# zhexin1904/gtsam_personal

Hardware: AMD Instinct MI355X
Metric: LM iterations/sec (higher is better)
Workload: dtype f64; 1 GPU; synthetic BAL 1000 cameras / 100000 points / 1000002 factors (GeneralSFMFactor<Cal3Bundler> + 2 priors), seed 42, METIS ordering (Ordering::Metis of the reference, fixture-carried permutation), LM legacy defaults; ordering=metis, cameras=1000, points=100000, factors=1000002, fronts=100001, parallelism=single GPU

## Files before the change

gtsam_personal_amd/_lib.py:

```python
from __future__ import annotations

import ctypes as ct
import os

_HERE = os.path.dirname(os.path.abspath(__file__))
LIB_PATH = os.path.join(_HERE, "liblmgpu.so")

LMGPU_OK, LMGPU_INDETERMINATE, LMGPU_INVALID, LMGPU_HIP_ERROR = 0, 1, 2, 3


class lmgpu_config(ct.Structure):
    _fields_ = [("device", ct.c_int32), ("rank", ct.c_int32), ("world_size", ct.c_int32), ("flags", ct.c_int32)]


class lmgpu_lm_params(ct.Structure):
    _fields_ = [
        ("maxIterations", ct.c_int32),
        ("relativeErrorTol", ct.c_double), ("absoluteErrorTol", ct.c_double), ("errorTol", ct.c_double),
        ("lambdaInitial", ct.c_double), ("lambdaFactor", ct.c_double), ("lambdaUpperBound", ct.c_double), ("lambdaLowerBound", ct.c_double),
        ("minModelFidelity", ct.c_double),
        ("diagonalDamping", ct.c_int32), ("useFixedLambdaFactor", ct.c_int32),
        ("minDiagonal", ct.c_double), ("maxDiagonal", ct.c_double),
    ]

# ... 128 lines not shown
    "lmgpu_init_pose3_num_factors": (ct.c_int, [_H]),
    "lmgpu_init_pose3_get_slots": (ct.c_int, [_H, ct.POINTER(ct.c_uint64)]),
    "lmgpu_init_pose3_handle": (ct.c_void_p, [_H, ct.c_int32]),
    "lmgpu_init_pose3_orientations_chordal": (ct.c_int, [_H, _D]),
    "lmgpu_init_pose3_closest_rotations": (ct.c_int, [ct.c_int32, ct.c_int32, _D, _D]),
    "lmgpu_init_pose3_orientations_gradient": (ct.c_int, [_H, _D, ct.c_int32, ct.c_int32, _D, _I, _D]),
    "lmgpu_init_pose3_compute_poses": (ct.c_int, [_H, _D, ct.c_int32, _D, ct.POINTER(lmgpu_lm_state)]),
    "lmgpu_init_pose3_initialize": (ct.c_int, [_H, _D, ct.c_int32, _D]),
    "lmgpu_set_kernel_timing": (ct.c_int, [_H, ct.c_int32]),
    "lmgpu_get_kernel_times": (ct.c_int, [_H, _D, _D, ct.POINTER(ct.c_int64)]),
    "lmgpu_get_jacobian": (ct.c_int, [_H, ct.c_int32, _D, _I, _I]),
    "lmgpu_get_jacobians": (ct.c_int, [_H, _I, _I, _I, _I, ct.POINTER(ct.c_int64), _D]),
    "lmgpu_num_fronts": (ct.c_int, [_H]),
    "lmgpu_front_info": (ct.c_int, [_H, ct.c_int32, _I]),
    "lmgpu_leaf_group_launches": (ct.c_int, [_H]),
    "lmgpu_backsub_group_launches": (ct.c_int, [_H, _I]),
    "lmgpu_get_leaf_corner": (ct.c_int, [_H, ct.c_int32, _D]),
    "lmgpu_get_front": (ct.c_int, [_H, ct.c_int32, _I, _D]),
    "lmgpu_comm_unique_id": (ct.c_int, [ct.c_char_p]),
    "lmgpu_comm_init": (ct.c_int, [_H, ct.c_char_p]),
    "lmgpu_marginal_covariance": (ct.c_int, [_H, ct.c_int32, _D]),
    "lmgpu_joint_marginal_covariance": (ct.c_int, [_H, ct.c_int32, _I, _D]),
    "lmgpu_selftest_chain_schedule": (ct.c_int, [ct.c_int, ct.c_int, ct.c_int, ct.c_int, ct.c_int]),
    "lmgpu_selftest_dense_schedule": (ct.c_int, [ct.c_int, ct.c_int, ct.c_int, ct.c_uint, ct.c_int, _I]),
    "lmgpu_selftest_dogleg_step": (ct.c_int, [ct.c_int, _D, _D]),
    "lmgpu_bt_products": (ct.c_int, [_H, _D, ct.c_double, _D, _D]),
    "lmgpu_isam2_create": (ct.c_int, [ct.POINTER(lmgpu_config), ct.c_void_p, ct.c_void_p, ct.c_void_p, ct.POINTER(_H)]),
    "lmgpu_isam2_destroy": (ct.c_int, [_H]),
    "lmgpu_isam2_last_error": (ct.c_char_p, [_H]),
    "lmgpu_isam2_last_failed_key": (ct.c_uint64, [_H]),
# ... 90 lines not shown
```

gtsam_personal_amd/csrc/kernels_potrf.hpp:

```cpp
#pragma once
#include <hip/hip_runtime.h>

namespace lmgpu {

typedef double double4_t __attribute__((ext_vector_type(4)));

__device__ __forceinline__ double readlane_d(double v, int src_lane) {
  const long long b = __double_as_longlong(v);
  const int lo = __builtin_amdgcn_readlane((int)(b & 0xffffffffLL), src_lane);
  const int hi = __builtin_amdgcn_readlane((int)(b >> 32), src_lane);
  return __longlong_as_double(((long long)hi << 32) | (unsigned int)lo);
}

__device__ __forceinline__ double fast_rsqrt(double p) {
  double y = __builtin_amdgcn_rsq(p);
  const double h = 0.5 * p;
  y = y * fma(-h * y, y, 1.5);
  y = y * fma(-h * y, y, 1.5);
  return y;
}

template <bool INV>
__device__ __forceinline__ bool potrf64_wave_g4(double4_t (&T)[4][4], double4_t (&E)[4], int nrows = 64) {
  const int lane = threadIdx.x & 63, kk = lane >> 4, cc = lane & 15;
  bool failed = false;
#pragma unroll
  for (int g = 0; g < 4; g++) {
    if (INV) {
#pragma unroll
      for (int r = 0; r < 4; r++) E[g][r] = (kk + 4 * r == cc) ? 1.0 : 0.0;
    }
    if (16 * g >= nrows) continue;
#pragma unroll
    for (int q = 0; q < 4; q++) {
      if (16 * g + 4 * q >= nrows) continue;
      double m[4][4];
#pragma unroll
      for (int a = 0; a < 4; a++)
#pragma unroll
        for (int b = a; b < 4; b++) m[a][b] = readlane_d(T[g][g][q], 16 * a + 4 * q + b);
      double R[4][4], inv[4];
#pragma unroll
      for (int a = 0; a < 4; a++) {
        double p = m[a][a];
#pragma unroll
        for (int k = 0; k < a; k++) p -= R[k][a] * R[k][a];
        const bool pok = p > 0.0;
        failed |= !pok;
        p = pok ? p : 1.0;
        const double rs = fast_rsqrt(p);
        inv[a] = rs;
        R[a][a] = p * rs;
#pragma unroll
        for (int b = a + 1; b < 4; b++) {
          double v = m[a][b];
#pragma unroll
          for (int k = 0; k < a; k++) v -= R[k][a] * R[k][b];
          R[a][b] = v * rs;
        }
      }
      double W[4][4];
#pragma unroll
      for (int a = 0; a < 4; a++) {
        W[a][a] = inv[a];
#pragma unroll
        for (int b = a + 1; b < 4; b++) {
          double v = 0;
#pragma unroll
          for (int k = a; k < b; k++) v += W[a][k] * R[k][b];
          W[a][b] = -v * inv[b];
        }
      }
      double aop = 0.0;
#pragma unroll
      for (int k = 0; k < 4; k++)
#pragma unroll
        for (int i = k; i < 4; i++) aop = (kk == k && cc == i) ? W[k][i] : aop;
      double bop = 0.0;
      {
        const double4_t x = __builtin_amdgcn_mfma_f64_16x16x4f64(aop, T[g][g][q], double4_t{0, 0, 0, 0}, 0, 0, 0);
        T[g][g][q] = x[0];
        if (q < 3) {
          bop = (cc >= 4 * (q + 1)) ? -T[g][g][q] : 0.0;
          T[g][g] = __builtin_amdgcn_mfma_f64_16x16x4f64(bop, T[g][g][q], T[g][g], 0, 0, 0);
        }
      }
#pragma unroll
      for (int h = g + 1; h < 4; h++) {
        const double4_t x = __builtin_amdgcn_mfma_f64_16x16x4f64(aop, T[g][h][q], double4_t{0, 0, 0, 0}, 0, 0, 0);
        T[g][h][q] = x[0];
        if (q < 3) T[g][h] = __builtin_amdgcn_mfma_f64_16x16x4f64(bop, T[g][h][q], T[g][h], 0, 0, 0);
      }
      if (INV) {
        const double4_t x = __builtin_amdgcn_mfma_f64_16x16x4f64(aop, E[g][q], double4_t{0, 0, 0, 0}, 0, 0, 0);
        E[g][q] = x[0];
        if (q < 3) E[g] = __builtin_amdgcn_mfma_f64_16x16x4f64(bop, E[g][q], E[g], 0, 0, 0);
      }
    }
#pragma unroll
    for (int g2 = g + 1; g2 < 4; g2++)
#pragma unroll
      for (int h = g2; h < 4; h++)
#pragma unroll
        for (int s = 0; s < 4; s++) T[g2][h] = __builtin_amdgcn_mfma_f64_16x16x4f64(-T[g][g2][s], T[g][h][s], T[g2][h], 0, 0, 0);
  }
  return failed;
}
__device__ __forceinline__ bool potrf64_wave_g4(double4_t (&T)[4][4]) {
  double4_t E[4];
  return potrf64_wave_g4<false>(T, E);
}

#define DP_LDW 66
#define DIAG_LDS_DOUBLES (64 * DP_LDW + 4 * 16 * 17 + 3 * 64 * DP_LDW)
#define DIAG_LDS_BYTES (DIAG_LDS_DOUBLES * 8)

__device__ __forceinline__ int frexp_exp_d(double x) {
  int e;
  frexp(x, &e);
// ... 206 lines not shown
          const int row = 16 * g + kk + 4 * r;
          if (row < nbj && cvalid) P[(size_t)(64 * j + row) * ld + c0 + cc] = out[r];
        }
      }
    }
  }
}

__global__ __launch_bounds__(256) void panel_trsm_kernel(double* __restrict__ A, int ld, int n, int ko, int kb, const double* __restrict__ inv16) {
  __shared__ double I16[16][16][17];
  panel_trsm_body(A, ld, n, ko, kb, inv16, I16, blockIdx.x);
}

#define TAIL_MAX_M 48
#define TAIL_MAX_KP 256
#define TAIL_LDS_BYTES ((TAIL_MAX_KP * TAIL_MAX_M + TAIL_MAX_M * TAIL_MAX_M + 64 * 65) * 8)
__global__ __launch_bounds__(256) void front_tail_kernel(double* __restrict__ A, int ld, int n, int nf, int p0, int kp, int front_id,
                                                         int* __restrict__ status, double* __restrict__ inv16) {
  extern __shared__ double tsm[];
  const int r0 = p0 + kp, m = n - r0, nft = nf - r0, tid = threadIdx.x;
  double* Pl = tsm;
  double* S = tsm + (size_t)TAIL_MAX_KP * TAIL_MAX_M;
  double(*D)[65] = (double(*)[65])(S + TAIL_MAX_M * TAIL_MAX_M);
  for (int idx = tid; idx < kp * m; idx += 256) {
    const int k = idx / m, j = idx - k * m;
    Pl[idx] = A[(size_t)(p0 + k) * ld + r0 + j];
  }
  for (int idx = tid; idx < m * m; idx += 256) {
    const int i = idx / m, j = idx - i * m;
    S[idx] = (j >= i) ? A[(size_t)(r0 + i) * ld + r0 + j] : 0.0;
  }
  __syncthreads();
  for (int idx = tid; idx < m * m; idx += 256) {
// ... 50 lines not shown
  __syncthreads();
  if (tid < 64) {
    const int blk = tid >> 4, c = tid & 15, base = 16 * blk;
    double x[16];
#pragma unroll
    for (int i = 15; i >= 0; i--) {
      double sacc = (i == c) ? 1.0 : 0.0;
#pragma unroll
      for (int kq = i + 1; kq < 16; kq++) sacc -= D[base + i][base + kq] * x[kq];
      x[i] = (i <= c) ? sacc / D[base + i][base + i] : 0.0;
    }
#pragma unroll
    for (int i = 0; i < 16; i++) inv16[(size_t)blk * 256 + i * 16 + c] = x[i];
  }
}

#ifndef PDF_STAMP
#define PDF_STAMP(flags, b, slot)
#endif
#define PDF_TA0 32
#define PDF_MAX_COLTILES 992
#define PDF_PR0 1024
#define PDF_TD0 1536
#define PDF_FLAG_WORDS 8192
#define PDF_MAX_CHAIN_T 114
#define PDF_SPIN_LIMIT 2000000L
#define PDF_LDS_DOUBLES (2 * 64 * DP_LDW)
#define PDF_LDS_BYTES (PDF_LDS_DOUBLES * 8)

__host__ __device__ inline unsigned int pdf_ta_need(int sj) { return sj < 4 ? 4u * (unsigned int)(sj + 1) : 2u; }
// ... 264 lines not shown
```

gtsam_personal_amd/csrc/lmgpu.hip:

```cpp
#include <hip/hip_runtime.h>
#include <rccl/rccl.h>

#include <algorithm>
#include <chrono>
#include <cmath>
#include <cstdio>
#include <cstdlib>
#include <cstring>
#include <condition_variable>
#include <limits>
#include <mutex>
#include <string>
#include <map>
#include <vector>

#include "../../include/lmgpu.h"
#include "kernels_dense.hpp"
#include "kernels_potrf.hpp"
#include "kernels_step.hpp"
#include "dense_schedule.hpp"
#include "dogleg_step.hpp"
#include "kernels_batched.hpp"
#include "kernels_level.hpp"
#include "kernels_bayes.hpp"
// ... 209 lines not shown
  LevelSync* d_level_sync = nullptr;
  int n_level_sync = 0;
  int32_t *d_bs_parent = nullptr, *d_bs_pos = nullptr;
  char* d_leafpack = nullptr;
  unsigned int* d_bs_done = nullptr;
  bool use_graph = false;
  int eager_solves = 0;
  hipGraphExec_t solve_graph[2] = {nullptr, nullptr};
  int leaf_group_threads = 256;
  bool no_backsub_groups = false;
  int n_leaf_group_launches = 0;
  bool no_wide16 = false;
  int wide16_max = 256;
  bool bsd_ticket = false;
  bool no_tail = false;
  bool no_chain = false;
  int chain_forms = 0;
  unsigned int* d_pflags = nullptr;
  int pflags_panels = 0;
  unsigned int* bs_flags = nullptr;
  double* pool = nullptr;
  size_t pool_doubles = 0;
  double* vals[2][kNumVarTypes] = {};
  double* saved[kNumVarTypes] = {};
  int cur = 0;
  int32_t* type_xoff[kNumVarTypes] = {};
  double *delta = nullptr, *dampw = nullptr, *hdiag = nullptr, *ebuf0 = nullptr, *ebuf1 = nullptr, *partial = nullptr, *dscal = nullptr,
         *ywork = nullptr;
  int* d_status = nullptr;
  double* h_scal = nullptr;
// ... 3 lines not shown
  FrontFac* d_ffac = nullptr;
  ChildRef* d_childs = nullptr;
  int32_t *d_cmap = nullptr, *d_fxoff = nullptr, *d_sxoff = nullptr, *d_lists = nullptr;
  int32_t *d_hbm_small = nullptr, *d_f_ld = nullptr, *d_med_list = nullptr;
  MedFront* d_med_fronts = nullptr;
  BsdBlock* d_bsd_table = nullptr;
  struct BsdRun {
    int lvl_hi, lvl_lo, begin, count;
  };
  std::vector<BsdRun> bsd_runs;
  std::vector<int> bsd_run_of;
  BsdBlock* d_bsd_run_table = nullptr;
  FillChunk* d_fill_elim = nullptr;
  FillChunk* d_fill_backsub = nullptr;
  int n_fill_elim = -1, n_fill_backsub = -1, fill_backsub_merge = -1;
  double* d_bsd_x = nullptr;
  unsigned int* d_bsd_ticket = nullptr;
  size_t bsd_x_count = 0;
  ZeroRange* d_zero_ranges = nullptr;
  int n_zero_ranges = 0;
  int num_cus = 0;
  std::vector<int32_t> row_begin;
  int32_t *d_row_begin = nullptr, *d_rowptr = nullptr;
  RowSrc* d_rowsrc = nullptr;
  int n_lds_fronts = 0;
  double *bt_ebuf = nullptr, *bt_vec = nullptr;
  int bt_ebuf_len = 0;
  double* bt_part = nullptr;
  int64_t* d_bt_part_off = nullptr;
  std::vector<int64_t> bt_hbm_part_off;
// ... 383 lines not shown
  h->dense_mode = mode;
  return LMGPU_OK;
}

int do_eliminate(lmgpu_handle* h, double lambda_v, const double* lambda_p) {
  hipStream_t s = h->stream;
  const bool merge_el = h->merge_elim && !h->elim_segs.empty();
  std::vector<FillChunk> fills;
  const bool build_fills = h->n_fill_elim < 0;
  if (build_fills) {
    add_fill(fills, h->d_status, sizeof(int), 0x7f7f7f7fu);
    add_fill(fills, h->d_status + 1, sizeof(int), 0u);
    if (merge_el || h->fuse_levels)
      add_fill(fills, h->d_bs_done, (size_t)(h->h_fronts.size() + h->levels.size() + 1) * sizeof(unsigned int), 0u);
    if (h->fuse_levels) add_fill(fills, h->d_level_sync, (size_t)h->n_level_sync * sizeof(LevelSync), 0u);
  }
  {
    const int kt0 = h->kt.begin(LMGPU_KT_HBM_ASSEMBLE, s);
    int n_hbm = 0;
    int64_t lo = INT64_MAX, hi = 0, sum = 0;
    for (const LevelWork& L : h->levels)
      for (int fi : L.hbm) {
        const int64_t cnt = (int64_t)h->h_fronts[fi].n * h->f_ld[fi] * (h->s_off[fi] >= 0 ? 2 : 1);
        n_hbm++;
        sum += cnt;
        lo = std::min(lo, h->f_off[fi]);
        hi = std::max(hi, h->f_off[fi] + cnt);
      }
    if (n_hbm > 4 && hi - lo <= 2 * sum) {
      if (build_fills) add_fill(fills, h->pool + lo, (size_t)(hi - lo) * sizeof(double), 0u);
// ... 16 lines not shown
    } else {
      for (const LevelWork& L : h->levels)
        for (int fi : L.hbm) {
          const bool gw = gather_writes(h, fi);
          const size_t bytes = (size_t)h->h_fronts[fi].n * h->f_ld[fi] * sizeof(double);
          if (!gw || h->s_off[fi] >= 0) HIPCHECK(hipMemsetAsync(h->pool + h->f_off[fi], 0, bytes, s));
          if (!gw && h->s_off[fi] >= 0) HIPCHECK(hipMemsetAsync(h->pool + h->s_off[fi], 0, bytes, s));
        }
    }
    if (build_fills) {
      h->n_fill_elim = (int)fills.size();
      const int rcu = upload(h, &h->d_fill_elim, fills);
      if (rcu) return rcu;
    }
    hipLaunchKernelGGL(fill_chunks_kernel, dim3(h->n_fill_elim), dim3(256), 0, s, (const FillChunk*)h->d_fill_elim);
    h->kt.end(kt0, s);
  }
  if (merge_el)
    hipLaunchKernelGGL(fill_upper_kernel, dim3(h->n_fill_upper), dim3(256), 0, s, (const FillUpper*)h->d_fill_upper, h->pool);
  for (size_t li = 0; li < h->levels.size(); li++) {
    const LevelWork& L = h->levels[li];
    const int seg = merge_el ? h->elim_seg_of[li] : -1;
    if (seg >= 0) {
      const lmgpu_handle::ElimSeg& E = h->elim_segs[seg];
      const int b0 = h->levels[E.lvl_lo].list_begin, e0 = h->levels[E.lvl_hi].list_begin + h->levels[E.lvl_hi].list_count;
      const size_t lds = kLdsFrontExtra - (size_t)(LDSF_JCAP - E.jcap) * 8 + 64 + (size_t)E.nmax * E.nmax * sizeof(double);
      const int kt = h->kt.begin(LMGPU_KT_LDS_FRONT, s);
      unsigned int* ticket = h->d_bs_done + h->h_fronts.size() + E.lvl_hi;
      auto* kernel = E.threads == 1024 ? lds_front_merged_kernel<1024> : lds_front_merged_kernel<256>;
      hipLaunchKernelGGL(kernel, dim3(e0 - b0), dim3(E.threads), lds, s, (const int32_t*)h->d_lists, b0, e0, (const FrontDesc*)h->d_fronts,
// ... 146 lines not shown
      h->inv16_owner = fi;
      int kt_run = -1, run_launches = 0;
      double run_flop = 0;
      for (size_t r = 0; r < plan.steps.size(); r++) {
        const DenseStep& st = plan.steps[r];
        const int i = st.i, k0 = i * NBO, kb = std::min(F.nf, k0 + NBO) - k0, r0 = k0 + kb, m = F.n - r0;
        const bool in_run = st.kind == DENSE_STEP_FUSED || (st.kind == DENSE_WAIT_CHUNK && plan.steps[r + 1].kind == DENSE_STEP_FUSED);
        if (!in_run && run_launches > 0) {
          h->kt.end(kt_run, s, run_flop, run_launches);
          run_launches = 0;
          run_flop = 0;
        }
        switch (st.kind) {
          case DENSE_PANEL_DATAFLOW:
          case DENSE_PANEL_TWO_LAUNCH: {
            if (i == 0) HIPCHECK(hipMemsetAsync(h->d_pflags, 0, (size_t)((F.nf + NBO - 1) / NBO + 1) * PDF_FLAG_WORDS * sizeof(unsigned int), s));
            double* inv16 = h->inv16 + (size_t)i * 4096;
            const int ktp = h->kt.begin(LMGPU_KT_PANEL, s);
            if (st.kind == DENSE_PANEL_DATAFLOW) {
              hipLaunchKernelGGL(panel_dataflow_kernel, dim3(kb / 64 + (m + 63) / 64), dim3(256), PDF_LDS_BYTES, s, A, ld, F.n, F.nf, k0, kb, F.id,
                                 h->d_status, inv16, h->d_pflags + (size_t)i * PDF_FLAG_WORDS);
            } else {
              hipLaunchKernelGGL(diag_potrf_kernel, dim3(1), dim3(256), DIAG_LDS_BYTES, s, A, ld, F.nf, k0, kb, F.id, h->d_status, inv16);
              if (m > 0) hipLaunchKernelGGL(panel_trsm_kernel, dim3((m + 63) / 64), dim3(256), 0, s, A, ld, F.n, k0, kb, (const double*)inv16);
            }
            h->kt.end(ktp, s, st.flop);
            break;
          }
          case DENSE_CHAIN: {
            ChainArgs ca{A, ld, F.n, F.nf, i, st.nsteps, F.id, h->d_status, h->inv16, h->d_pflags, h->d_chain_tasks + plan.task_begin[r],
                         split ? (const double*)Asm : nullptr};
// ... 21 lines not shown
          case DENSE_UPDATE_QUADRANTS:
          case DENSE_UPDATE_MFMA: {
            const int kts = h->kt.begin(LMGPU_KT_SYRK, s);
            if (st.kind == DENSE_UPDATE_QUADRANTS) {
              const int S = (m + 63) / 64;
              hipLaunchKernelGGL(syrk_quadrants_kernel, dim3(4 * S, S), dim3(256), 0, s, A, ld, F.n, k0, kb, r0);
            } else {
              const int T = (m + 127) / 128;
              hipLaunchKernelGGL(syrk_mfma_kernel, dim3(T, T), dim3(256), kSyrkLds, s, A, ld, F.n, k0, kb, r0, F.n);
            }
            h->kt.end(kts, s, st.flop);
            break;
          }
          case DENSE_TAIL: {
            const int ktt = h->kt.begin(LMGPU_KT_PANEL, s);
            hipLaunchKernelGGL(front_tail_kernel, dim3(1), dim3(256), TAIL_LDS_BYTES, s, A, ld, F.n, F.nf, k0, kb, F.id, h->d_status,
                               h->inv16 + (size_t)(i + 1) * 4096);
            h->kt.end(ktt, s, st.flop);
            break;
          }
          case DENSE_ADD_CHUNK:
          case DENSE_WAIT_CHUNK: {
            const int rcc = st.kind == DENSE_ADD_CHUNK ? add_chunk(h, A, Asm, F.n, ld, st.chunk) : wait_chunk(h, Asm, F.n, ld, st.chunk);
            if (rcc) return rcc;
            break;
          }
        }
      }
      if (run_launches > 0) h->kt.end(kt_run, s, run_flop, run_launches);
    }
  }
  HIPCHECK(hipGetLastError());
// ... 136 lines not shown
      h->kt.end(kt, s);
    }
    for (int fi : L.hbm) {
      const FrontDesc& F = h->h_fronts[fi];
      if (F.nf <= BSS_MAX_NF) continue;
      const int64_t off = h->f_off[fi];
      const int ld = h->f_ld[fi];
      const int kt = h->kt.begin(LMGPU_KT_BACKSUB_HBM, s);
      const bool has_sep = F.n - F.nf - 1 > 0;
      if (has_sep)
        hipLaunchKernelGGL(hbm_rhs_init_kernel, dim3(F.nf), dim3(64), 0, s, F, off, ld, (const int32_t*)h->d_sxoff, (const double*)h->pool,
                           (const double*)h->delta, h->ywork);
      const bool reuse = h->inv16_owner == fi && !dev_switch("LMGPU_NO_INV16_REUSE");
      const bool wide = reuse && !dev_switch("LMGPU_BACKSOLVE_HOP64");
      const int bw = wide ? BSW_NB : NB, nblk = (F.nf + bw - 1) / bw;
      HIPCHECK(hipMemsetAsync(h->bs_flags, 0, (nblk + 1) * sizeof(unsigned int), s));
      HIPCHECK(hipMemsetAsync(h->bs_x, 0xff, (size_t)nblk * bw * sizeof(double), s));
      if (wide) {
        hipLaunchKernelGGL((hbm_backsolve_wide_kernel<false>), dim3(nblk), dim3(512), 0, s, F, off, ld, (const int32_t*)h->d_fxoff, (const double*)h->pool,
                           (const double*)h->inv16, has_sep ? (const double*)h->ywork : (const double*)nullptr, h->bs_x, h->bs_flags, h->delta,
                           h->d_status, h->bs_inv, (unsigned long long*)nullptr);
#ifdef LMGPU_TEST_HOOKS
      } else if (reuse) {
        hipLaunchKernelGGL((hbm_backsolve_dataflow2_kernel<false>), dim3(nblk), dim3(256), 0, s, F, off, ld, (const int32_t*)h->d_fxoff, (const double*)h->pool,
                           (const double*)h->inv16, has_sep ? (const double*)h->ywork : (const double*)nullptr, h->bs_x, h->bs_flags, h->delta,
                           h->d_status, (unsigned long long*)nullptr);
#endif
      } else {
        if (!has_sep)
          hipLaunchKernelGGL(hbm_rhs_init_kernel, dim3(F.nf), dim3(64), 0, s, F, off, ld, (const int32_t*)h->d_sxoff, (const double*)h->pool,
                             (const double*)h->delta, h->ywork);
        hipLaunchKernelGGL((hbm_invert_diag_kernel<NB>), dim3(nblk), dim3(NB), 0, s, (const double*)(h->pool + off), ld, F.nf, h->bs_inv);
// ... 688 lines not shown
}

extern "C" {

int lmgpu_create(const lmgpu_config* cfg, lmgpu_handle** out) {
  if (!cfg || !out) return LMGPU_INVALID;
  lmgpu_handle* h = new lmgpu_handle();
  h->cfg = *cfg;
  if (h->cfg.world_size < 1) h->cfg.world_size = 1;
  h->device = cfg->device;
  h->two_launch_panel = dev_switch("LMGPU_PANEL_2L") != nullptr;
  h->no_fuse = dev_switch("LMGPU_NO_FUSE") != nullptr;
  h->no_chain = dev_switch("LMGPU_NO_CHAIN") != nullptr;
  h->chain_forms = (dev_switch("LMGPU_CHAIN_FENCED_TILES") ? CHAIN_FORM_FENCED_TILES : 0) | (dev_switch("LMGPU_CHAIN_PREREAD") ? CHAIN_FORM_PREREAD : 0);
  h->no_tail = dev_switch("LMGPU_NO_TAIL") != nullptr;
  h->no_wide16 = dev_switch("LMGPU_NO_WIDE16") != nullptr;
  if (const char* e = dev_switch("LMGPU_LEAF_GROUP_THREADS")) h->leaf_group_threads = atoi(e) == 64 ? 64 : (atoi(e) == 128 ? 128 : 256);
  h->no_backsub_groups = dev_switch("LMGPU_NO_BACKSUB_GROUPS") != nullptr;
  if (const char* e = dev_switch("LMGPU_WIDE16_MAX")) h->wide16_max = atoi(e);
  h->bsd_ticket = dev_switch("LMGPU_BSD_TICKET") != nullptr;
  h->no_gather_write = dev_switch("LMGPU_NO_GATHER_WRITE") != nullptr;
  h->schur_split_diag = dev_switch("LMGPU_SCHUR_SPLIT_DIAG") != nullptr;
  h->pcg_fused = dev_switch("LMGPU_PCG_FUSED") != nullptr;
  if (dev_switch("LMGPU_NO_MERGE")) h->chain_merge = false;
  if (const char* e = dev_switch("LMGPU_CHAIN_SPLIT")) h->chain_split_pct = std::max(0, std::min(100, atoi(e)));
  if (const char* e = dev_switch("LMGPU_CHAIN_FAR")) h->chain_far_pct = std::max(10, std::min(100, atoi(e)));
  *out = h;
  if (h->device >= 0) {
    HIPCHECK(hipSetDevice(h->device));
    {
// ... 15 lines not shown
    HIPCHECK(hipMemset(h->d_lambda, 0, sizeof(double)));
    HIPCHECK(hipFuncSetAttribute((const void*)lds_front_kernel<false>, hipFuncAttributeMaxDynamicSharedMemorySize, kLdsLimitN * kLdsLimitN * 8 + kLdsFrontExtra + 64));
    HIPCHECK(hipFuncSetAttribute((const void*)lds_front_kernel<false, 1024>, hipFuncAttributeMaxDynamicSharedMemorySize, kLdsLimitN * kLdsLimitN * 8 + kLdsFrontExtra + 64));
    HIPCHECK(hipFuncSetAttribute((const void*)lds_front_kernel<true>, hipFuncAttributeMaxDynamicSharedMemorySize, kLdsLimitN * kLdsLimitN * 8 + kLdsFrontExtra + 64));
    HIPCHECK(hipFuncSetAttribute((const void*)lds_front_merged_kernel<256>, hipFuncAttributeMaxDynamicSharedMemorySize, kLdsLimitN * kLdsLimitN * 8 + kLdsFrontExtra + 64));
    HIPCHECK(hipFuncSetAttribute((const void*)lds_front_merged_kernel<1024>, hipFuncAttributeMaxDynamicSharedMemorySize, kLdsLimitN * kLdsLimitN * 8 + kLdsFrontExtra + 64));
    HIPCHECK(hipFuncSetAttribute((const void*)level_fused_kernel<256>, hipFuncAttributeMaxDynamicSharedMemorySize, kLdsLimitN * kLdsLimitN * 8 + kLdsFrontExtra + 64));
    HIPCHECK(hipFuncSetAttribute((const void*)level_fused_kernel<1024>, hipFuncAttributeMaxDynamicSharedMemorySize, kLdsLimitN * kLdsLimitN * 8 + kLdsFrontExtra + 64));
    HIPCHECK(hipFuncSetAttribute((const void*)syrk_mfma_kernel, hipFuncAttributeMaxDynamicSharedMemorySize, kSyrkLds));
    HIPCHECK(hipFuncSetAttribute((const void*)lds_backsub_wide_kernel, hipFuncAttributeMaxDynamicSharedMemorySize, (kLdsLimitN * kLdsLimitN + LDSB_TAIL) * 8));
    HIPCHECK(hipFuncSetAttribute((const void*)lds_backsub_merged_kernel, hipFuncAttributeMaxDynamicSharedMemorySize, (kLdsLimitN * kLdsLimitN + LDSB_TAIL) * 8));
    HIPCHECK(hipFuncSetAttribute((const void*)diag_potrf_kernel, hipFuncAttributeMaxDynamicSharedMemorySize, DIAG_LDS_BYTES));
    HIPCHECK(hipFuncSetAttribute((const void*)panel_dataflow_kernel, hipFuncAttributeMaxDynamicSharedMemorySize, PDF_LDS_BYTES));
    HIPCHECK(hipFuncSetAttribute((const void*)step_kernel, hipFuncAttributeMaxDynamicSharedMemorySize, STEP_LDS_BYTES));
    HIPCHECK(hipFuncSetAttribute((const void*)chain_kernel, hipFuncAttributeMaxDynamicSharedMemorySize, STEP_LDS_BYTES));
    HIPCHECK(hipFuncSetAttribute((const void*)front_tail_kernel, hipFuncAttributeMaxDynamicSharedMemorySize, TAIL_LDS_BYTES));
    HIPCHECK(hipFuncSetAttribute((const void*)med_diag_potrf_kernel, hipFuncAttributeMaxDynamicSharedMemorySize, DIAG_LDS_BYTES));
  }
  return LMGPU_OK;
}

int lmgpu_destroy(lmgpu_handle* h) {
  if (!h) return LMGPU_INVALID;
  if (h->device >= 0) {
    (void)hipSetDevice(h->device);
    if (h->stream) (void)hipStreamSynchronize(h->stream);
    if (h->comm_data) ncclCommDestroy(h->comm_data);
    if (h->comm) ncclCommDestroy(h->comm);
    auto fr = [](void* p) {
      if (p) (void)hipFree(p);
    };
// ... 882 lines not shown
  if ((rc = upload(h, &h->d_gpent, gpent))) return rc;
  if ((rc = upload(h, &h->d_gvblk, gvblk))) return rc;
  if ((rc = upload(h, &h->d_gvent, gvent))) return rc;
  HIPCHECK(hipMalloc((void**)&h->d_gcorner, std::max<size_t>(1, (size_t)n_gleaf) * sizeof(double)));
  if ((rc = finalize_vectors(h))) return rc;
  {
    int max_nf = 1;
    for (int fi = 0; fi < NF; fi++)
      if (h->front_active[fi] && P.fronts[fi].cls == 1) max_nf = std::max(max_nf, P.fronts[fi].nf);
    const int max_blk = (max_nf + NB - 1) / NB;
    HIPCHECK(hipMalloc((void**)&h->bs_inv, (size_t)((max_nf + BSW_NB - 1) / BSW_NB) * BSW_NB * BSW_NB * sizeof(double)));
    HIPCHECK(hipMalloc((void**)&h->inv16, (size_t)((P.max_front_n + NBO - 1) / NBO + 2) * 16 * 256 * sizeof(double)));
    h->pflags_panels = (P.max_front_n + NBO - 1) / NBO + 1;
    HIPCHECK(hipMalloc((void**)&h->d_pflags, (size_t)h->pflags_panels * PDF_FLAG_WORDS * sizeof(unsigned int)));

    HIPCHECK(hipMalloc((void**)&h->bs_x, (size_t)((max_nf + BSW_NB - 1) / BSW_NB) * BSW_NB * sizeof(double)));
    HIPCHECK(hipMalloc((void**)&h->bs_flags, (size_t)(max_blk + 1) * sizeof(unsigned int)));
  }
  return LMGPU_OK;
}

int lmgpu_total_dim(const lmgpu_handle* h) { return (h && h->finalized) ? h->ntot : -1; }
int lmgpu_total_store(const lmgpu_handle* h) { return (h && h->finalized) ? h->nstore : -1; }

int lmgpu_set_values(lmgpu_handle* h, const double* packed) {
  if (!h) return LMGPU_INVALID;
  if (!h->finalized || !packed) {
    h->err = "lmgpu_set_values: refused (!h->finalized || !packed)";
    return LMGPU_INVALID;
  }
  int rc = need_device(h);
  if (rc) return rc;
// ... 906 lines not shown
    const Bucket& b = h->buckets[f.bucket];
    const size_t sz = (size_t)b.rows * b.cols;
    if (b.loc_of[f.idx] < 0) {
      h->err = "lmgpu_get_jacobians: a factor lives on another rank";
      return LMGPU_INVALID;
    }
    std::memcpy(out + off, jb[f.bucket].data() + (size_t)b.loc_of[f.idx] * sz, sz * sizeof(double));
    off += (int64_t)sz;
  }
  return LMGPU_OK;
}

int lmgpu_num_fronts(const lmgpu_handle* h) { return (h && h->finalized) ? (int)h->plan.fronts.size() : -1; }

int lmgpu_leaf_group_launches(const lmgpu_handle* h) { return (h && h->finalized) ? h->n_leaf_group_launches : -1; }

int lmgpu_backsub_group_launches(const lmgpu_handle* h, int32_t* wide) {
  if (!h || !h->finalized) return -1;
  int cnt = 0, w = 0;
  for (const LevelWork& L : h->levels) {
    const int form = backsub_group_form(h, L);
    cnt += form != 0;
    w += form == 2;
  }
  if (wide) *wide = w;
  return cnt;
}

int lmgpu_get_leaf_corner(lmgpu_handle* h, int32_t front, double* corner) {
  if (!h) return LMGPU_INVALID;
// ... 417 lines not shown
```

gtsam_personal_amd/optimizer.py:

```python
from __future__ import annotations

import ctypes as ct

import numpy as np

from . import _lib
from .graph import (CAM_BUNDLER, F_PRIOR_CAM, F_SFM, FACTOR_ARITY, N_UNIT, VAR_DIM, VAR_STORE, VAR_STORE_DEV, NonlinearFactorGraph, Ordering,
                    Values)


class DummyPreconditionerParameters:
    kind = _lib.LMGPU_PRECOND_DUMMY


class BlockJacobiPreconditionerParameters:
    kind = _lib.LMGPU_PRECOND_BLOCK_JACOBI


class PCGSolverParameters:

    def __init__(self, preconditioner=None):
        self.minIterations = 1
        self.maxIterations = 500
        self.reset = 501
# ... 313 lines not shown
        return (None if xp is None else sq.value), g

    def jacobian(self, graph_index):
        r, c = ct.c_int32(), ct.c_int32()
        self._check(self.lib.lmgpu_get_jacobian(self._h, graph_index, None, ct.byref(r), ct.byref(c)))
        out = np.empty(r.value * c.value)
        self._check(self.lib.lmgpu_get_jacobian(self._h, graph_index, _dp(out), ct.byref(r), ct.byref(c)))
        return out.reshape(c.value, r.value).T.copy()

    def num_fronts(self):
        return self.lib.lmgpu_num_fronts(self._h)

    def leaf_group_launches(self):
        return self.lib.lmgpu_leaf_group_launches(self._h)

    def backsub_group_launches(self):
        wide = np.zeros(1, dtype=np.int32)
        return self.lib.lmgpu_backsub_group_launches(self._h, _ip(wide)), int(wide[0])

    def leaf_corner(self, i):
        out = np.zeros(1)
        self._check(self.lib.lmgpu_get_leaf_corner(self._h, i, _dp(out)))
        return float(out[0])

    def front_info(self, i):
        info = np.zeros(8, dtype=np.int32)
        self._check(self.lib.lmgpu_front_info(self._h, i, _ip(info)))
        return dict(n_keys=int(info[0]), n_frontal_keys=int(info[1]), nf=int(info[2]), n=int(info[3]), parent=int(info[4]), cls=int(info[5]),
                    owner=int(info[6]), level=int(info[7]))

# ... 445 lines not shown
```

include/lmgpu.h:

```cpp
#ifndef LMGPU_H
#define LMGPU_H
#include <stdint.h>

#ifdef __cplusplus
extern "C" {
#endif

typedef struct lmgpu_handle lmgpu_handle;

enum lmgpu_status {
  LMGPU_OK = 0,
  LMGPU_INDETERMINATE = 1,
  LMGPU_INVALID = 2,
  LMGPU_HIP_ERROR = 3
};

enum lmgpu_var_type {
  LMGPU_POSE2 = 0,
  LMGPU_POSE3 = 1,
  LMGPU_POINT3 = 2,
  LMGPU_CAM_BUNDLER = 3,
  LMGPU_POINT2 = 4,
  LMGPU_CAL3_S2 = 5,
  LMGPU_VEC9 = 6,
// ... 184 lines not shown
  LMGPU_KT_BACKSUB_LDS = 6,
  LMGPU_KT_LINEAR_ERROR = 7,
  LMGPU_KT_RETRACT_ERROR = 8,
  LMGPU_KT_ALLREDUCE = 9,
  LMGPU_KT_CHAIN = 10,
  LMGPU_KT_NUM = 11
};
int lmgpu_set_kernel_timing(lmgpu_handle* h, int32_t on);
int lmgpu_get_kernel_times(const lmgpu_handle* h, double* ms , double* work , int64_t* launches );

int lmgpu_get_jacobian(lmgpu_handle* h, int32_t graph_index, double* out, int32_t* rows, int32_t* cols);
int lmgpu_get_jacobians(lmgpu_handle* h, int32_t* n_out, int32_t* graph_index, int32_t* rows, int32_t* cols, int64_t* offsets, double* out);
int lmgpu_num_fronts(const lmgpu_handle* h);
int lmgpu_front_info(const lmgpu_handle* h, int32_t front, int32_t* info8);
int lmgpu_leaf_group_launches(const lmgpu_handle* h);
int lmgpu_backsub_group_launches(const lmgpu_handle* h, int32_t* wide);
int lmgpu_get_leaf_corner(lmgpu_handle* h, int32_t front, double* corner);
int lmgpu_get_front(lmgpu_handle* h, int32_t front, int32_t* slots, double* RSd_colmajor);

int lmgpu_comm_unique_id(char id128[128]);
int lmgpu_comm_init(lmgpu_handle* h, const char id128[128]);

int lmgpu_marginal_covariance(lmgpu_handle* h, int32_t slot, double* cov );
int lmgpu_joint_marginal_covariance(lmgpu_handle* h, int32_t nslots, const int32_t* slots, double* cov );

int lmgpu_selftest_chain_schedule(int n, int nf, int i0, int nsteps, int far_pct);

int lmgpu_selftest_dense_schedule(int n, int nf, int mode, unsigned forms, int max_records, int32_t* out);

int lmgpu_selftest_dogleg_step(int which, const double* in, double* out);
// ... 76 lines not shown
```

Baseline: 141.8 LM iterations/s.

## Rewrite front tail factorization with MFMA register tiles and fold memsets into fill

After: 142.9 LM iterations/s (median of 6 runs). About the same (+0.7%).

```diff
diff --git a/gtsam_personal_amd/_lib.py b/gtsam_personal_amd/_lib.py
--- a/gtsam_personal_amd/_lib.py
+++ b/gtsam_personal_amd/_lib.py
@@ -166,6 +166,7 @@
     "lmgpu_num_fronts": (ct.c_int, [_H]),
     "lmgpu_front_info": (ct.c_int, [_H, ct.c_int32, _I]),
     "lmgpu_leaf_group_launches": (ct.c_int, [_H]),
+    "lmgpu_tail_launches": (ct.c_int, [_H, ct.POINTER(ct.c_int32)]),
     "lmgpu_backsub_group_launches": (ct.c_int, [_H, _I]),
     "lmgpu_get_leaf_corner": (ct.c_int, [_H, ct.c_int32, _D]),
     "lmgpu_get_front": (ct.c_int, [_H, ct.c_int32, _I, _D]),
diff --git a/gtsam_personal_amd/csrc/kernels_potrf.hpp b/gtsam_personal_amd/csrc/kernels_potrf.hpp
--- a/gtsam_personal_amd/csrc/kernels_potrf.hpp
+++ b/gtsam_personal_amd/csrc/kernels_potrf.hpp
@@ -20,12 +20,13 @@
   return y;
 }
 
-template <bool INV>
-__device__ __forceinline__ bool potrf64_wave_g4(double4_t (&T)[4][4], double4_t (&E)[4], int nrows = 64) {
+template <bool INV, int NS = 4, bool PARTIAL = false>
+__device__ __forceinline__ bool potrf64_wave_g4(double4_t (&T)[4][4], double4_t (&E)[4], int nrows = 64, int npiv = 64) {
   const int lane = threadIdx.x & 63, kk = lane >> 4, cc = lane & 15;
   bool failed = false;
-#pragma unroll
-  for (int g = 0; g < 4; g++) {
+  if (PARTIAL) nrows = min(nrows, npiv);
+#pragma unroll
+  for (int g = 0; g < NS; g++) {
     if (INV) {
 #pragma unroll
       for (int r = 0; r < 4; r++) E[g][r] = (kk + 4 * r == cc) ? 1.0 : 0.0;
@@ -34,6 +35,7 @@
 #pragma unroll
     for (int q = 0; q < 4; q++) {
       if (16 * g + 4 * q >= nrows) continue;
+      const int np = PARTIAL ? nrows - (16 * g + 4 * q) : 4;
       double m[4][4];
 #pragma unroll
       for (int a = 0; a < 4; a++)
@@ -45,10 +47,11 @@
         double p = m[a][a];
 #pragma unroll
         for (int k = 0; k < a; k++) p -= R[k][a] * R[k][a];
+        const bool pivot = !PARTIAL || a < np;
         const bool pok = p > 0.0;
-        failed |= !pok;
-        p = pok ? p : 1.0;
-        const double rs = fast_rsqrt(p);
+        failed |= PARTIAL ? (pivot && p <= 0.0) : !pok;
+        p = (pok && pivot) ? p : 1.0;
+        const double rs = pivot ? fast_rsqrt(p) : 1.0;
         inv[a] = rs;
         R[a][a] = p * rs;
 #pragma unroll
@@ -56,7 +59,7 @@
           double v = m[a][b];
 #pragma unroll
           for (int k = 0; k < a; k++) v -= R[k][a] * R[k][b];
-          R[a][b] = v * rs;
+          R[a][b] = pivot ? v * rs : 0.0;
         }
       }
       double W[4][4];
@@ -81,12 +84,12 @@
         const double4_t x = __builtin_amdgcn_mfma_f64_16x16x4f64(aop, T[g][g][q], double4_t{0, 0, 0, 0}, 0, 0, 0);
         T[g][g][q] = x[0];
         if (q < 3) {
-          bop = (cc >= 4 * (q + 1)) ? -T[g][g][q] : 0.0;
+          bop = (cc >= 4 * (q + 1) && (!PARTIAL || kk < np)) ? -T[g][g][q] : 0.0;
           T[g][g] = __builtin_amdgcn_mfma_f64_16x16x4f64(bop, T[g][g][q], T[g][g], 0, 0, 0);
         }
       }
 #pragma unroll
-      for (int h = g + 1; h < 4; h++) {
+      for (int h = g + 1; h < NS; h++) {
         const double4_t x = __builtin_amdgcn_mfma_f64_16x16x4f64(aop, T[g][h][q], double4_t{0, 0, 0, 0}, 0, 0, 0);
         T[g][h][q] = x[0];
         if (q < 3) T[g][h] = __builtin_amdgcn_mfma_f64_16x16x4f64(bop, T[g][h][q], T[g][h], 0, 0, 0);
@@ -97,12 +100,20 @@
         if (q < 3) E[g] = __builtin_amdgcn_mfma_f64_16x16x4f64(bop, E[g][q], E[g], 0, 0, 0);
       }
     }
-#pragma unroll
-    for (int g2 = g + 1; g2 < 4; g2++)
-#pragma unroll
-      for (int h = g2; h < 4; h++)
-#pragma unroll
-        for (int s = 0; s < 4; s++) T[g2][h] = __builtin_amdgcn_mfma_f64_16x16x4f64(-T[g][g2][s], T[g][h][s], T[g2][h], 0, 0, 0);
+    if (PARTIAL && INV) {
+#pragma unroll
+      for (int r = 0; r < 4; r++)
+        if (16 * g + kk + 4 * r >= nrows) E[g][r] = (kk + 4 * r == cc) ? 1.0 : 0.0;
+    }
+#pragma unroll
+    for (int g2 = g + 1; g2 < NS; g2++)
+#pragma unroll
+      for (int h = g2; h < NS; h++)
+#pragma unroll
+        for (int s = 0; s < 4; s++) {
+          const double a = (!PARTIAL || 16 * g + 4 * s + kk < nrows) ? -T[g][g2][s] : 0.0;
+          T[g2][h] = __builtin_amdgcn_mfma_f64_16x16x4f64(a, T[g][h][s], T[g2][h], 0, 0, 0);
+        }
   }
   return failed;
 }
@@ -339,9 +350,110 @@
 
 #define TAIL_MAX_M 48
 #define TAIL_MAX_KP 256
-#define TAIL_LDS_BYTES ((TAIL_MAX_KP * TAIL_MAX_M + TAIL_MAX_M * TAIL_MAX_M + 64 * 65) * 8)
+#define TAIL_NT ((TAIL_MAX_M + 15) / 16)
+#define TAIL_TILES (TAIL_NT * (TAIL_NT + 1) / 2)
 __global__ __launch_bounds__(256) void front_tail_kernel(double* __restrict__ A, int ld, int n, int nf, int p0, int kp, int front_id,
                                                          int* __restrict__ status, double* __restrict__ inv16) {
+  __shared__ double red[3][TAIL_TILES][4][64];
+  __shared__ double dg[16 * TAIL_NT];
+  __shared__ int s_failed;
+  const int r0 = p0 + kp, m = n - r0, nft = nf - r0, tid = threadIdx.x, wave = tid >> 6, lane = tid & 63, kk = lane >> 4, cc = lane & 15;
+  const int nt = (m + 15) >> 4;
+  const int ksteps = kp >> 2, sbeg = (ksteps * wave) >> 2, send = (ksteps * (wave + 1)) >> 2;
+  double4_t acc[TAIL_NT][TAIL_NT];
+#pragma unroll
+  for (int g = 0; g < TAIL_NT; g++)
+#pragma unroll
+    for (int h = g; h < TAIL_NT; h++) {
+#pragma unroll
+      for (int r = 0; r < 4; r++) {
+        const int row = 16 * g + kk + 4 * r, col = 16 * h + cc;
+        double v = (row == col) ? 1.0 : 0.0;
+        if (wave == 0 && row < m && col < m) v = A[(size_t)(r0 + row) * ld + r0 + col];
+        acc[g][h][r] = (wave == 0) ? v : 0.0;
+      }
+    }
+  const double* Pw = A + (size_t)p0 * ld + r0;
+  for (int s0 = sbeg; s0 < send; s0 += 16) {
+    double f[16][TAIL_NT];
+#pragma unroll
+    for (int s = 0; s < 16; s++)
+#pragma unroll
+      for (int t = 0; t < TAIL_NT; t++) {
+        const int k = 4 * (s0 + s) + kk, col = 16 * t + cc;
+        const bool ok = s0 + s < send && t < nt && col < m;
+        const double v = (s0 + s < send && t < nt) ? Pw[(size_t)k * ld + min(col, m - 1)] : 0.0;
+        f[s][t] = ok ? v : 0.0;
+      }
+#pragma unroll
+    for (int s = 0; s < 16; s++)
+#pragma unroll
+      for (int g = 0; g < TAIL_NT; g++)
+#pragma unroll
+        for (int h = g; h < TAIL_NT; h++)
+          acc[g][h] = __builtin_amdgcn_mfma_f64_16x16x4f64(-f[s][g], f[s][h], acc[g][h], 0, 0, 0);
+  }
+  if (wave > 0) {
+    int x = 0;
+#pragma unroll
+    for (int g = 0; g < TAIL_NT; g++)
+#pragma unroll
+      for (int h = g; h < TAIL_NT; h++, x++)
+#pragma unroll
+        for (int r = 0; r < 4; r++) red[wave - 1][x][r][lane] = acc[g][h][r];
+  }
+  if (tid == 0) s_failed = 0;
+  __syncthreads();
+  if (wave == 0) {
+    double4_t T[4][4], E[4];
+    int x = 0;
+#pragma unroll
+    for (int g = 0; g < TAIL_NT; g++)
+#pragma unroll
+      for (int h = g; h < TAIL_NT; h++, x++)
+#pragma unroll
+        for (int r = 0; r < 4; r++) T[g][h][r] = (acc[g][h][r] + red[0][x][r][lane]) + (red[1][x][r][lane] + red[2][x][r][lane]);
+    const bool failed = potrf64_wave_g4<true, TAIL_NT, true>(T, E, 16 * TAIL_NT, nft);
+#pragma unroll
+    for (int g = 0; g < TAIL_NT; g++)
+#pragma unroll
+      for (int r = 0; r < 4; r++) {
+        const int row = 16 * g + kk + 4 * r;
+#pragma unroll
+        for (int h = g; h < TAIL_NT; h++) {
+          const int col = 16 * h + cc;
+          if (row < m && col < m && col >= row) A[(size_t)(r0 + row) * ld + r0 + col] = T[g][h][r];
+        }
+        if (kk + 4 * r == cc) dg[row] = T[g][g][r];
+        inv16[(size_t)g * 256 + cc * 16 + kk + 4 * r] = E[g][r];
+      }
+#pragma unroll
+    for (int g = TAIL_NT; g < 4; g++)
+#pragma unroll
+      for (int r = 0; r < 4; r++) inv16[(size_t)g * 256 + cc * 16 + kk + 4 * r] = (kk + 4 * r == cc) ? 1.0 : 0.0;
+    if (failed && lane == 0) s_failed = 1;
+  }
+  __syncthreads();
+  if (tid == 0) {
+    bool failed = s_failed != 0;
+    if (nft >= 2) {
+      if (!(frexp_exp_d(dg[nft - 2]) - frexp_exp_d(dg[nft - 1]) < 12)) failed = true;
+    } else if (nft == 1) {
+      const double r1 = dg[0];
+      if (nf >= 2) {
+        if (!(frexp_exp_d(A[(size_t)(nf - 2) * ld + nf - 2]) - frexp_exp_d(r1) < 12)) failed = true;
+      } else if (!(frexp_exp_d(r1) > -12)) {
+        failed = true;
+      }
+    }
+    if (failed) atomicMin(status, front_id);
+  }
+}
+
+#ifdef LMGPU_TEST_HOOKS
+#define TAIL_LDS_BYTES ((TAIL_MAX_KP * TAIL_MAX_M + TAIL_MAX_M * TAIL_MAX_M + 64 * 65) * 8)
+__global__ __launch_bounds__(256) void front_tail_scalar_kernel(double* __restrict__ A, int ld, int n, int nf, int p0, int kp, int front_id,
+                                                                int* __restrict__ status, double* __restrict__ inv16) {
   extern __shared__ double tsm[];
   const int r0 = p0 + kp, m = n - r0, nft = nf - r0, tid = threadIdx.x;
   double* Pl = tsm;
@@ -422,6 +534,7 @@
     for (int i = 0; i < 16; i++) inv16[(size_t)blk * 256 + i * 16 + c] = x[i];
   }
 }
+#endif
 
 #ifndef PDF_STAMP
 #define PDF_STAMP(flags, b, slot)
diff --git a/gtsam_personal_amd/csrc/lmgpu.hip b/gtsam_personal_amd/csrc/lmgpu.hip
--- a/gtsam_personal_amd/csrc/lmgpu.hip
+++ b/gtsam_personal_amd/csrc/lmgpu.hip
@@ -247,6 +247,8 @@
   int wide16_max = 256;
   bool bsd_ticket = false;
   bool no_tail = false;
+  bool tail_scalar = false;
+  int n_tail_launches[2] = {0, 0};
   bool no_chain = false;
   int chain_forms = 0;
   unsigned int* d_pflags = nullptr;
@@ -280,6 +282,9 @@
   FillChunk* d_fill_elim = nullptr;
   FillChunk* d_fill_backsub = nullptr;
   int n_fill_elim = -1, n_fill_backsub = -1, fill_backsub_merge = -1;
+  int pflags_fill_front = -1;
+  bool elim_arms_bs = false, bs_armed = false;
+  size_t bs_x_bytes = 0, bs_flags_bytes = 0;
   double* d_bsd_x = nullptr;
   unsigned int* d_bsd_ticket = nullptr;
   size_t bsd_x_count = 0;
@@ -693,6 +698,22 @@
     if (merge_el || h->fuse_levels)
       add_fill(fills, h->d_bs_done, (size_t)(h->h_fronts.size() + h->levels.size() + 1) * sizeof(unsigned int), 0u);
     if (h->fuse_levels) add_fill(fills, h->d_level_sync, (size_t)h->n_level_sync * sizeof(LevelSync), 0u);
+    h->pflags_fill_front = -1;
+    for (size_t li = 0; li < h->levels.size() && h->pflags_fill_front < 0; li++)
+      for (int fi : h->levels[li].hbm)
+        if (!h->is_med[fi]) {
+          h->pflags_fill_front = fi;
+          break;
+        }
+    if (h->pflags_fill_front >= 0)
+      add_fill(fills, h->d_pflags, (size_t)((h->h_fronts[h->pflags_fill_front].nf + NBO - 1) / NBO + 1) * PDF_FLAG_WORDS * sizeof(unsigned int), 0u);
+    h->elim_arms_bs = false;
+    for (const LevelWork& L : h->levels)
+      for (int fi : L.hbm) h->elim_arms_bs |= h->h_fronts[fi].nf > BSS_MAX_NF;
+    if (h->elim_arms_bs) {
+      add_fill(fills, h->bs_flags, h->bs_flags_bytes, 0u);
+      add_fill(fills, h->bs_x, h->bs_x_bytes, 0xffffffffu);
+    }
   }
   {
     const int kt0 = h->kt.begin(LMGPU_KT_HBM_ASSEMBLE, s);
@@ -739,6 +760,7 @@
       if (rcu) return rcu;
     }
     hipLaunchKernelGGL(fill_chunks_kernel, dim3(h->n_fill_elim), dim3(256), 0, s, (const FillChunk*)h->d_fill_elim);
+    h->bs_armed = h->elim_arms_bs;
     h->kt.end(kt0, s);
   }
   if (merge_el)
@@ -915,7 +937,8 @@
         switch (st.kind) {
           case DENSE_PANEL_DATAFLOW:
           case DENSE_PANEL_TWO_LAUNCH: {
-            if (i == 0) HIPCHECK(hipMemsetAsync(h->d_pflags, 0, (size_t)((F.nf + NBO - 1) / NBO + 1) * PDF_FLAG_WORDS * sizeof(unsigned int), s));
+            if (i == 0 && fi != h->pflags_fill_front)
+              HIPCHECK(hipMemsetAsync(h->d_pflags, 0, (size_t)((F.nf + NBO - 1) / NBO + 1) * PDF_FLAG_WORDS * sizeof(unsigned int), s));
             double* inv16 = h->inv16 + (size_t)i * 4096;
             const int ktp = h->kt.begin(LMGPU_KT_PANEL, s);
             if (st.kind == DENSE_PANEL_DATAFLOW) {
@@ -967,8 +990,18 @@
           }
           case DENSE_TAIL: {
             const int ktt = h->kt.begin(LMGPU_KT_PANEL, s);
-            hipLaunchKernelGGL(front_tail_kernel, dim3(1), dim3(256), TAIL_LDS_BYTES, s, A, ld, F.n, F.nf, k0, kb, F.id, h->d_status,
-                               h->inv16 + (size_t)(i + 1) * 4096);
+#ifdef LMGPU_TEST_HOOKS
+            if (h->tail_scalar) {
+              hipLaunchKernelGGL(front_tail_scalar_kernel, dim3(1), dim3(256), TAIL_LDS_BYTES, s, A, ld, F.n, F.nf, k0, kb, F.id, h->d_status,
+                                 h->inv16 + (size_t)(i + 1) * 4096);
+              h->n_tail_launches[1]++;
+            } else
+#endif
+            {
+              hipLaunchKernelGGL(front_tail_kernel, dim3(1), dim3(256), 0, s, A, ld, F.n, F.nf, k0, kb, F.id, h->d_status,
+                                 h->inv16 + (size_t)(i + 1) * 4096);
+              h->n_tail_launches[0]++;
+            }
             h->kt.end(ktt, s, st.flop);
             break;
           }
@@ -1135,8 +1168,11 @@
       const bool reuse = h->inv16_owner == fi && !dev_switch("LMGPU_NO_INV16_REUSE");
       const bool wide = reuse && !dev_switch("LMGPU_BACKSOLVE_HOP64");
       const int bw = wide ? BSW_NB : NB, nblk = (F.nf + bw - 1) / bw;
-      HIPCHECK(hipMemsetAsync(h->bs_flags, 0, (nblk + 1) * sizeof(unsigned int), s));
-      HIPCHECK(hipMemsetAsync(h->bs_x, 0xff, (size_t)nblk * bw * sizeof(double), s));
+      if (!h->bs_armed) {
+        HIPCHECK(hipMemsetAsync(h->bs_flags, 0, (nblk + 1) * sizeof(unsigned int), s));
+        HIPCHECK(hipMemsetAsync(h->bs_x, 0xff, (size_t)nblk * bw * sizeof(double), s));
+      }
+      h->bs_armed = false;
       if (wide) {
         hipLaunchKernelGGL((hbm_backsolve_wide_kernel<false>), dim3(nblk), dim3(512), 0, s, F, off, ld, (const int32_t*)h->d_fxoff, (const double*)h->pool,
                            (const double*)h->inv16, has_sep ? (const double*)h->ywork : (const double*)nullptr, h->bs_x, h->bs_flags, h->delta,
@@ -1855,6 +1891,7 @@
   h->no_chain = dev_switch("LMGPU_NO_CHAIN") != nullptr;
   h->chain_forms = (dev_switch("LMGPU_CHAIN_FENCED_TILES") ? CHAIN_FORM_FENCED_TILES : 0) | (dev_switch("LMGPU_CHAIN_PREREAD") ? CHAIN_FORM_PREREAD : 0);
   h->no_tail = dev_switch("LMGPU_NO_TAIL") != nullptr;
+  h->tail_scalar = dev_switch("LMGPU_TAIL_SCALAR") != nullptr;
   h->no_wide16 = dev_switch("LMGPU_NO_WIDE16") != nullptr;
   if (const char* e = dev_switch("LMGPU_LEAF_GROUP_THREADS")) h->leaf_group_threads = atoi(e) == 64 ? 64 : (atoi(e) == 128 ? 128 : 256);
   h->no_backsub_groups = dev_switch("LMGPU_NO_BACKSUB_GROUPS") != nullptr;
@@ -1900,7 +1937,9 @@
     HIPCHECK(hipFuncSetAttribute((const void*)panel_dataflow_kernel, hipFuncAttributeMaxDynamicSharedMemorySize, PDF_LDS_BYTES));
     HIPCHECK(hipFuncSetAttribute((const void*)step_kernel, hipFuncAttributeMaxDynamicSharedMemorySize, STEP_LDS_BYTES));
     HIPCHECK(hipFuncSetAttribute((const void*)chain_kernel, hipFuncAttributeMaxDynamicSharedMemorySize, STEP_LDS_BYTES));
-    HIPCHECK(hipFuncSetAttribute((const void*)front_tail_kernel, hipFuncAttributeMaxDynamicSharedMemorySize, TAIL_LDS_BYTES));
+#ifdef LMGPU_TEST_HOOKS
+    HIPCHECK(hipFuncSetAttribute((const void*)front_tail_scalar_kernel, hipFuncAttributeMaxDynamicSharedMemorySize, TAIL_LDS_BYTES));
+#endif
     HIPCHECK(hipFuncSetAttribute((const void*)med_diag_potrf_kernel, hipFuncAttributeMaxDynamicSharedMemorySize, DIAG_LDS_BYTES));
   }
   return LMGPU_OK;
@@ -2813,8 +2852,10 @@
     h->pflags_panels = (P.max_front_n + NBO - 1) / NBO + 1;
     HIPCHECK(hipMalloc((void**)&h->d_pflags, (size_t)h->pflags_panels * PDF_FLAG_WORDS * sizeof(unsigned int)));
 
-    HIPCHECK(hipMalloc((void**)&h->bs_x, (size_t)((max_nf + BSW_NB - 1) / BSW_NB) * BSW_NB * sizeof(double)));
-    HIPCHECK(hipMalloc((void**)&h->bs_flags, (size_t)(max_blk + 1) * sizeof(unsigned int)));
+    h->bs_x_bytes = (size_t)((max_nf + BSW_NB - 1) / BSW_NB) * BSW_NB * sizeof(double);
+    h->bs_flags_bytes = (size_t)(max_blk + 1) * sizeof(unsigned int);
+    HIPCHECK(hipMalloc((void**)&h->bs_x, h->bs_x_bytes));
+    HIPCHECK(hipMalloc((void**)&h->bs_flags, h->bs_flags_bytes));
   }
   return LMGPU_OK;
 }
@@ -3751,6 +3792,11 @@
 int lmgpu_num_fronts(const lmgpu_handle* h) { return (h && h->finalized) ? (int)h->plan.fronts.size() : -1; }
 
 int lmgpu_leaf_group_launches(const lmgpu_handle* h) { return (h && h->finalized) ? h->n_leaf_group_launches : -1; }
+int lmgpu_tail_launches(const lmgpu_handle* h, int32_t* scalar) {
+  if (!h || !h->finalized) return -1;
+  if (scalar) *scalar = h->n_tail_launches[1];
+  return h->n_tail_launches[0];
+}
 
 int lmgpu_backsub_group_launches(const lmgpu_handle* h, int32_t* wide) {
   if (!h || !h->finalized) return -1;
diff --git a/gtsam_personal_amd/optimizer.py b/gtsam_personal_amd/optimizer.py
--- a/gtsam_personal_amd/optimizer.py
+++ b/gtsam_personal_amd/optimizer.py
@@ -351,6 +351,10 @@
     def leaf_group_launches(self):
         return self.lib.lmgpu_leaf_group_launches(self._h)
 
+    def tail_launches(self):
+        scalar = np.zeros(1, dtype=np.int32)
+        return self.lib.lmgpu_tail_launches(self._h, _ip(scalar)), int(scalar[0])
+
     def backsub_group_launches(self):
         wide = np.zeros(1, dtype=np.int32)
         return self.lib.lmgpu_backsub_group_launches(self._h, _ip(wide)), int(wide[0])
diff --git a/include/lmgpu.h b/include/lmgpu.h
--- a/include/lmgpu.h
+++ b/include/lmgpu.h
@@ -222,6 +222,7 @@
 int lmgpu_num_fronts(const lmgpu_handle* h);
 int lmgpu_front_info(const lmgpu_handle* h, int32_t front, int32_t* info8);
 int lmgpu_leaf_group_launches(const lmgpu_handle* h);
+int lmgpu_tail_launches(const lmgpu_handle* h, int32_t* scalar);
 int lmgpu_backsub_group_launches(const lmgpu_handle* h, int32_t* wide);
 int lmgpu_get_leaf_corner(lmgpu_handle* h, int32_t front, double* corner);
 int lmgpu_get_front(lmgpu_handle* h, int32_t front, int32_t* slots, double* RSd_colmajor);
```
